# dcjones/polee

Hardware: AMD Instinct MI355X
Metric: approx-lik VI iters/sec (higher is better)
Workload: dtype f32

## Files before the change

### include/polee_hip_debug.h

```cpp
#ifndef POLEE_HIP_DEBUG_H
#define POLEE_HIP_DEBUG_H

#include "polee_hip.h"

#ifdef __cplusplus
extern "C" {
#endif

polee_status polee_debug_ptt_plan(const int32_t *node_parent_idxs, const int32_t *node_js, int32_t N,
                                  uint32_t *tour_code, int32_t *tour_tgt, int32_t *leaf_tid,
                                  int32_t *lo, int32_t *mid, int32_t *hi1, int32_t *max_depth);

typedef struct polee_psell_debug polee_psell_debug;
typedef struct {
    int64_t m, n, nnz, num_slices, num_tiles, padded_nnz, num_empty_rows;
    int64_t data_bytes, dict_len;
    int32_t max_row_nnz, max_tile_cols;
    const uint8_t *data;
    const uint32_t *slice_off;
    const uint32_t *tile_slice;
    const uint32_t *tile_dict;
    const uint32_t *dict;
    const uint32_t *row_order;
    const float *slice_ks;
    const uint8_t *slice_flags;
    int64_t num_tiles_a;
    int64_t num_tiles_a1;
    int64_t num_tiles_a1m;
    int64_t num_tiles_a2;
    const uint8_t *slice_w;
    int64_t num_tiles_s;
    int64_t stream_rows[8], stream_nnz[8], stream_bytes[8];
    int64_t csr_num_rows;
    const uint32_t *csr_rowptr;
    const uint32_t *csr_col;
    const float *csr_val;
    const uint32_t *csr_rows;
    int64_t single_num_rows;
    const uint32_t *single_rows;
    const float *single_cnt;
    double single_logsum;
} polee_psell_view;
polee_status polee_debug_psell_build(int64_t m, int64_t n, const void *colptr, int colptr_bytes,
                                     const uint32_t *rowval, const float *nzval,
                                     const int64_t *ks_or_null, polee_psell_debug **out);
polee_status polee_debug_psell_build_device(polee_ctx *ctx, int64_t m, int64_t n, const void *colptr, int colptr_bytes,
                                            const uint32_t *rowval, const float *nzval, const int64_t *ks_or_null,
                                            int device_stages, polee_psell_debug **out);
polee_status polee_debug_psell_view(const polee_psell_debug *p, polee_psell_view *view);
void polee_debug_psell_free(polee_psell_debug *p);

void polee_debug_device_cache_poison(int64_t *checked_blocks, int64_t *bad_blocks, int64_t *bad_words);

polee_status polee_debug_loglik_force_mixed(polee_loglik *ll, int on);

int64_t polee_debug_regression_num_stats(const polee_regression *reg);
polee_status polee_debug_regression_data_pass(polee_regression *reg, const float *noise, float *stats);
polee_status polee_debug_regression_prior_pass(polee_regression *reg, const float *stats, float *loss,
                                               float *grad_or_null);

polee_status polee_debug_comm_allreduce_ms(polee_comm *comm, int64_t count, int32_t reps, double *ms_avg);

polee_status polee_debug_fast_log(polee_ctx *ctx, const double *x, int64_t count, double *out);
polee_status polee_debug_fast_exp(polee_ctx *ctx, const double *x, int64_t count, double *out);

polee_status polee_debug_gibbs_assignments(polee_gibbs *g, int32_t chain, int32_t *z);

#ifdef __cplusplus
}
#endif
#endif
```

### polee_amd/csrc/loglik.hip

```cpp
#include "loglik_internal.hpp"
#include "psell_device.hpp"
#include "wave.hpp"

#include <algorithm>
#include <chrono>
#include <cmath>
#include <queue>
#include <type_traits>

namespace polee {

template <int CTRL, int ROW_MASK>
__device__ inline float dpp_mov0(float v)
{
    return __int_as_float(__builtin_amdgcn_update_dpp(0, __float_as_int(v), CTRL, ROW_MASK, 0xf, true));
}

template <int K>
__device__ inline void scatter_runs(int c, float (&q)[K], float *gw, int lane)
{
    const int c0 = __builtin_amdgcn_readfirstlane(c);
    if (__all(c == c0)) {
        float *gr = gw + c0 * K;
        wave_sum_to_lane63_n<K>(q);
// ... 66 lines not shown
    }
    __device__ inline void mul(float s, bool valid)
    {
        const float sv = valid ? s : 1.0f;
        const float p = m * __builtin_amdgcn_frexp_mantf(sv);
        m = __builtin_amdgcn_frexp_mantf(p);
        e += __builtin_amdgcn_frexp_expf(sv) + __builtin_amdgcn_frexp_expf(p);
    }
    __device__ inline double log_value() const { return ((double)e + (double)__builtin_amdgcn_logf(m)) * 0.693147180559945309417; }
};
__device__ inline double ks_log2(float ksv, float s) { return (double)(ksv * __builtin_amdgcn_logf(s)); }

struct PsellArgs {
    const uint8_t *data;
    const uint32_t *slice_off, *tile_slice, *tile_dict, *dict;
    const float *slice_ks;
    const float *x;
    float *g;
    double *lp;
    int lcap;
    int tiles_a;
    int tiles_a1;
    int tiles_a1m, tiles_a2;
    int tiles_s;
    const float *xwin;
    const PosDesc *sched;
    const PosDesc *sched_dyn;
    unsigned int *dyn_ctr;
    unsigned int dyn_base;
    unsigned int dyn_last;
    float *gwin;
    double *lpwin;
    int lp_slot0;
};

template <int K, bool WANT_LP, bool HAS_KS>
__device__ inline void psell_tile_body(const PsellArgs &A, int tile, float *xw, float *gw, double *lp_red)
{
    const uint8_t *__restrict__ data = A.data;
    const uint32_t *__restrict__ slice_off = A.slice_off;
    const uint32_t *__restrict__ tile_slice = A.tile_slice;
    const uint32_t *__restrict__ tile_dict = A.tile_dict;
    const uint32_t *__restrict__ dict = A.dict;
    const float *__restrict__ slice_ks = A.slice_ks;
    const float *__restrict__ x = A.x;
    float *__restrict__ g = A.g;
    double *__restrict__ lp = A.lp;

    const uint32_t d0 = tile_dict[tile];
    const int L = (int)(tile_dict[tile + 1] - d0);
    for (int i = threadIdx.x; i < L * K; i += 256) {
        const int l = i / K, k = i - l * K;
        xw[i] = x[(size_t)dict[d0 + l] * K + k];
        gw[i] = 0.0f;
    }
    __syncthreads();

    const int lane = threadIdx.x & 63, wave = threadIdx.x >> 6;
    const uint32_t s0 = tile_slice[tile], s1 = tile_slice[tile + 1];
    const bool compact = tile < A.tiles_a;
    double lpacc[K];
#pragma unroll
    for (int k = 0; k < K; ++k) lpacc[k] = 0.0;

    const int stream = tile < A.tiles_a1 ? PSELL_A1 : (tile < A.tiles_a1m ? PSELL_A1M : (tile < A.tiles_a2 ? PSELL_A2 : (tile < A.tiles_a ? PSELL_A2M : (tile < A.tiles_s ? PSELL_BN : PSELL_B))));
    const bool det = A.gwin != nullptr && tile >= A.tiles_s;
// ... 222 lines not shown
    return l;
}

__device__ inline void lds_barrier()
{
    asm volatile("s_waitcnt lgkmcnt(0)\n\ts_barrier" ::: "memory");
}

#ifdef POLEE_STAMPS
__device__ unsigned long long g_stamps[24];

#define STAMP(i)                                                          \
    do {                                                                  \
        const unsigned long long now__ = __builtin_amdgcn_s_memtime();    \
        st_acc[i] += now__ - st_last;                                     \
        st_last = now__;                                                  \
    } while (0)
#else
#define STAMP(i) do { } while (0)
#endif
#ifdef POLEE_TILE_CYCLES
__device__ unsigned long long g_tile_cycles[1 << 17];
__device__ unsigned long long g_wg_cycles[4096];
#endif
constexpr int NSTAMP = 16;

struct WaveStream {
    uint32_t ent;
    int nsl;
    int npieces;
    int issued, islot;
    int primed;
    const uint8_t *gsrc;
};

template <uint32_t RB>
__device__ inline void ring_refill(WaveStream &ws, uint32_t ring_lds, int target)
{
    constexpr int RP = (int)(RB / 1024u);
    int issued = __builtin_amdgcn_readfirstlane(ws.issued), islot = __builtin_amdgcn_readfirstlane(ws.islot);
    target = __builtin_amdgcn_readfirstlane(target);
    const uint32_t voff = (uint32_t)wave_lane() * 16u;
    const uint8_t *src = reinterpret_cast<const uint8_t *>(uniform_ptr(ws.gsrc + (size_t)issued * 1024));
    for (; issued < target; ++issued) {
        dma_1k(src, voff, ring_lds + (uint32_t)islot * 1024u);
        src += 1024;
        islot = islot + 1 == RP ? 0 : islot + 1;
    }
    ws.issued = issued;
    ws.islot = islot;
}

template <int K, uint32_t RB, bool WANT_LP, bool HAS_KS>
__device__ inline void wide_stream(WaveStream &ws, const char *ring, int extras, const float *xw, float *gw, double &lpacc, int dbg
#ifdef POLEE_STAMPS
                                   , unsigned long long (&st_acc)[NSTAMP], unsigned long long &st_last
#endif
                                   )
{
    constexpr int RP = (int)(RB / 1024u);
    constexpr uint32_t STAGE_A = 256u + 16u * 256u;
    static_assert(STAGE_A + 2046u <= RB && (PSELL_WIDE_MAX - 16 + 1) * 256u + 2046u <= RB, "a stage of a wide slice (+ ks row) must fit the ring");
    const int lane = wave_lane();
    const uint32_t ring_lds = lds_addr(ring);

    typedef float f32x4 __attribute__((ext_vector_type(4)));
    constexpr int NT = 2;
    constexpr int NS = 8;
    const int tt = lane & 15, q = lane >> 4;
    f32x4 acc0[NT], acc1[NT];
    uint2 colq[NT];
    float xq[NS];
#pragma unroll
    for (int mt = 0; mt < NT; ++mt) {
        acc0[mt] = f32x4{0.f, 0.f, 0.f, 0.f};
        acc1[mt] = f32x4{0.f, 0.f, 0.f, 0.f};
        colq[mt] = make_uint2(0u, 0u);
    }
#pragma unroll
    for (int st = 0; st < NS; ++st) xq[st] = 0.0f;
    int pend_w = 0;
    LogAcc lpl;
    lpl.init();
// ... 179 lines not shown
    const uint64_t E = 0x5555555555555555ull, L = 0x3333333333333333ull;
    asm volatile("s_nop 1\n\t"
                 "s_mov_b64 vcc, %8\n\t"
                 "v_cndmask_b32_dpp %4, %1, %0, vcc quad_perm:[1,0,3,2] row_mask:0xf bank_mask:0xf\n\t"
                 "v_cndmask_b32_dpp %6, %3, %2, vcc quad_perm:[1,0,3,2] row_mask:0xf bank_mask:0xf\n\t"
                 "s_not_b64 vcc, vcc\n\t"
                 "v_cndmask_b32_dpp %5, %0, %1, vcc quad_perm:[1,0,3,2] row_mask:0xf bank_mask:0xf\n\t"
                 "v_cndmask_b32_dpp %7, %2, %3, vcc quad_perm:[1,0,3,2] row_mask:0xf bank_mask:0xf\n\t"
                 "s_mov_b64 vcc, %9\n\t"
                 "v_cndmask_b32_dpp %0, %6, %4, vcc quad_perm:[2,3,0,1] row_mask:0xf bank_mask:0xf\n\t"
                 "v_cndmask_b32_dpp %1, %7, %5, vcc quad_perm:[2,3,0,1] row_mask:0xf bank_mask:0xf\n\t"
                 "s_not_b64 vcc, vcc\n\t"
                 "v_cndmask_b32_dpp %2, %4, %6, vcc quad_perm:[2,3,0,1] row_mask:0xf bank_mask:0xf\n\t"
                 "v_cndmask_b32_dpp %3, %5, %7, vcc quad_perm:[2,3,0,1] row_mask:0xf bank_mask:0xf"
                 : "+v"(a0), "+v"(a1), "+v"(a2), "+v"(a3), "=&v"(y0), "=&v"(y1), "=&v"(y2), "=&v"(y3)
                 : "s"(E), "s"(L)
                 : "vcc", "scc");
}

template <int K, uint32_t RB, bool WANT_LP, bool HAS_KS, bool MASKED>
__device__ inline void narrow_stream(WaveStream &ws, const char *ring, int extras, const float *xw, float *gw,
                                     uint32_t aux_lds, double &lpacc, int dbg
#ifdef POLEE_STAMPS
                                     , unsigned long long (&st_acc)[NSTAMP], unsigned long long &st_last
#endif
                                     )
{
    typedef float f32x4 __attribute__((ext_vector_type(4)));
    typedef const __attribute__((address_space(3))) float *lds_cfp;
    typedef __attribute__((address_space(3))) float *lds_fp;
    constexpr int WMAX = PSELL_NARROW_MAX;
    static_assert(WMAX == 16, "four groups of four transcripts");
    constexpr int KG = (K + 3) / 4;
    constexpr int RP = (int)(RB / 1024u);
    const int lane = wave_lane();
    const uint32_t ring_lds = lds_addr(ring);
    const uint32_t xw_lds = lds_addr(xw), gw_lds = lds_addr(gw);
    const int j = lane & 3, b = lane >> 2;
    const uint32_t j4 = 4u * (uint32_t)j;
    uint32_t lc1[4];
#pragma unroll
    for (int u = 0; u < 4; ++u) lc1[u] = ring_lds + ((uint32_t)(lane ^ u) << 2);
    const uint32_t j256 = 256u * (uint32_t)j;
    auto lds_f = [](uint32_t a) -> float { return *reinterpret_cast<lds_cfp>((uintptr_t)a); };
    auto wrap_u = [&](uint32_t a) -> uint32_t {
        a = (uint32_t)__builtin_amdgcn_readfirstlane((int)a);
        return a >= RB ? a - RB : a;
    };

    f32x4 acc[4][KG];
    float xq[8][KG];
#pragma unroll
    for (int g = 0; g < 4; ++g)
#pragma unroll
        for (int kg = 0; kg < KG; ++kg) acc[g][kg] = f32x4{0.f, 0.f, 0.f, 0.f};
#pragma unroll
    for (int t = 0; t < 8; ++t)
#pragma unroll
        for (int kg = 0; kg < KG; ++kg) xq[t][kg] = 0.0f;
    uint32_t xav = aux_lds, gav = aux_lds + 32u;
    int pend_w = 0;
    int run_w = 0;
    LogAcc lpl[KG];
    double lp2[KG];
#pragma unroll
    for (int kg = 0; kg < KG; ++kg) {
        lpl[kg].init();
// ... 6 lines not shown
        const uint32_t ga = ((lane & 32) ? ((lane & 16) ? ga3 : ga1) : ((lane & 16) ? ga2 : ga0)) + j4;
#pragma unroll
        for (int kg = 0; kg < KG; ++kg) {
            auto r1 = __builtin_amdgcn_permlane32_swap(__float_as_uint(acc[g][kg][0]), __float_as_uint(acc[g][kg][1]), false, false);
            const float ab = __uint_as_float(r1[0]) + __uint_as_float(r1[1]);
            auto r2 = __builtin_amdgcn_permlane32_swap(__float_as_uint(acc[g][kg][2]), __float_as_uint(acc[g][kg][3]), false, false);
            const float cd = __uint_as_float(r2[0]) + __uint_as_float(r2[1]);
            auto r3 = __builtin_amdgcn_permlane16_swap(__float_as_uint(ab), __float_as_uint(cd), false, false);
            float q = __uint_as_float(r3[0]) + __uint_as_float(r3[1]);
            q += __int_as_float(__builtin_amdgcn_update_dpp(0, __float_as_int(q), 0x114, 0xf, 0xf, true));
            q += __int_as_float(__builtin_amdgcn_update_dpp(0, __float_as_int(q), 0x118, 0xf, 0xf, true));
            if ((lane & 12) == 12 && 4 * kg + j < K && !(dbg & 2))
                __hip_atomic_fetch_add(reinterpret_cast<lds_fp>((uintptr_t)(ga + 16u * (uint32_t)kg)), q, __ATOMIC_RELAXED,
                                       __HIP_MEMORY_SCOPE_WORKGROUP);
            acc[g][kg] = f32x4{0.f, 0.f, 0.f, 0.f};
        }
    };
    auto flush = [&]() {
        flush_group(0);
        if (pend_w > 4) flush_group(1);
        if (pend_w > 8) flush_group(2);
        if (pend_w > 12) flush_group(3);
        pend_w = 0;
    };
    auto load_x_group = [&](int g, float (*dst)[KG]) {
#pragma unroll
        for (int u = 0; u < 4; ++u) {
            const uint32_t a = (uint32_t)__builtin_amdgcn_readlane((int)xav, 4 * g + u) + j4;
            dst[u][0] = lds_f(a);
            if (KG > 1) dst[u][KG > 1 ? 1 : 0] = lds_f(a + 16u);
        }
    };

    uint32_t pos = 0;
    uint32_t pos_r = 0;
    for (int si = 0; si < ws.nsl; ++si) {
        const uint32_t e0 = (uint32_t)__builtin_amdgcn_readlane((int)ws.ent, si);
        const uint32_t e1 = (uint32_t)__builtin_amdgcn_readlane((int)ws.ent, si + 1);
        const uint32_t off = e0 & PSELL_OFF_MASK, off_next = e1 & PSELL_OFF_MASK;
        const int flags = (int)(e0 >> 30);
        const uint32_t units = off_next - off;
        const int nrows = (int)(units / 2u) - 1 - (HAS_KS ? 1 : 0);
        int w = MASKED ? run_w : nrows;
        const uint32_t bytes = units * 128u;
        if (!(dbg & 16)) __builtin_amdgcn_s_setprio(3);
        STAMP(1);
        {
            const int need = (int)((pos + bytes + 1023u) >> 10);
            int allowed = ws.issued - need + (need <= ws.primed ? extras : 0);
            wait_vm_outstanding(__builtin_amdgcn_readfirstlane(allowed));
        }
        STAMP(2);
        if (pend_w != 0 && !(flags & 2)) flush();
        if (pend_w == 0 && !((dbg & 64) && si > 0)) {
            const uint32_t cid = *reinterpret_cast<const __attribute__((address_space(3))) uint16_t *>(
                (uintptr_t)(ring_lds + pos_r + (MASKED ? 4u * (uint32_t)(lane & 15) + 2u : 2u * (uint32_t)(lane & 15))));
            const bool live = MASKED ? cid != (uint32_t)PSELL_NO_COL : (lane & 15) < w;
            if (MASKED) {
                run_w = __builtin_popcount((uint32_t)__ballot(live) & 0xffffu);
                w = run_w;
            }
            xav = live ? xw_lds + cid * (uint32_t)(K * 4) : aux_lds;
            gav = live ? gw_lds + cid * (uint32_t)(K * 4) : aux_lds + 32u;
            load_x_group(0, xq);
            if (w > 4) load_x_group(1, xq + 4);
        }
        STAMP(3);

        const uint32_t row0 = wrap_u(pos_r + 256u);
        f32x4 d1[KG];
#pragma unroll
        for (int kg = 0; kg < KG; ++kg) d1[kg] = f32x4{ROWSUM_FLOOR, ROWSUM_FLOOR, ROWSUM_FLOOR, ROWSUM_FLOOR};
        f32x4 kv = f32x4{1.f, 1.f, 1.f, 1.f};
        auto consumed = [&]() {
            asm volatile("s_waitcnt lgkmcnt(0)" ::: "memory");
            STAMP(11);
            pos += bytes;
            pos_r += bytes;
            pos_r = pos_r >= RB ? pos_r - RB : pos_r;
            ring_refill<RB>(ws, ring_lds, min(ws.npieces, (int)(pos >> 10) + RP));
            STAMP(6);
            if (!(dbg & 16)) __builtin_amdgcn_s_setprio(0);
        };
        auto body = [&](auto NGc, auto FASTc) {
            constexpr int NG = decltype(NGc)::value;
            constexpr bool FAST = decltype(FASTc)::value;
            float pv[8], qv[2][4];
            uint32_t bp[4];
            if (FAST) {
#pragma unroll
                for (int u = 0; u < 4; ++u) bp[u] = lc1[u] + pos_r;
            }
            auto read_p = [&](int g0, int g1) {
#pragma unroll
                for (int g = g0; g < g1; ++g) {
                    if (FAST) {
#pragma unroll
                        for (int u = 0; u < 4; ++u) pv[4 * (g - g0) + u] = lds_f(bp[u] + 256u + 1024u * (uint32_t)g + 256u * (uint32_t)u);
                    } else {
                        const uint32_t rg = wrap_u(row0 + 1024u * (uint32_t)g);
#pragma unroll
                        for (int u = 0; u < 4; ++u) pv[4 * (g - g0) + u] = lds_f(lc1[u] + wrap_u(rg + 256u * (uint32_t)u));
                    }
                }
            };
            auto read_q = [&](int g0, int g1) {
#pragma unroll
                for (int g = g0; g < g1; ++g) {
                    if (FAST) {
#pragma unroll
                        for (int u = 0; u < 4; ++u) qv[g - g0][u] = lds_f(bp[u] + j256 + 256u + 1024u * (uint32_t)g);
                    } else {
                        const uint32_t rg = wrap_u(row0 + 1024u * (uint32_t)g);
// ... 81 lines not shown
                for (int u = 0; u < 8; ++u) pw[u] = pv[u];
                read_p(2, NG);
                if (!(dbg & 4)) {
                    load_x_group(2, xr);
                    if (NG > 3) load_x_group(3, xr + 4);
                } else {
#pragma unroll
                    for (int u = 0; u < 8; ++u)
#pragma unroll
                        for (int kg = 0; kg < KG; ++kg) xr[u][kg] = xq[u][kg];
                }
                asm volatile("s_waitcnt lgkmcnt(0)" ::: "memory");
                if (!(dbg & 16)) __builtin_amdgcn_s_setprio(0);
                phase1(pw, xq);
                phase1(pw + 4, xq + 4);
                phase1(pv, xr);
                if (NG > 3) phase1(pv + 4, xr + 4);
                read_q(0, 2);
#pragma unroll
                for (int u = 0; u < 4; ++u) {
                    qw[0][u] = qv[0][u];
                    qw[1][u] = qv[1][u];
                }
                read_q(2, NG);
                weights();
                consumed();
                phase2(0, qw[0]);
                phase2(1, qw[1]);
                phase2(2, qv[0]);
                if (NG > 3) phase2(3, qv[1]);
            }
        };
        using std::integral_constant;
        const bool fast = pos_r + bytes <= RB;
        if (fast) {
            if (w <= 4) body(integral_constant<int, 1>(), integral_constant<bool, true>());
            else if (w <= 8) body(integral_constant<int, 2>(), integral_constant<bool, true>());
            else if (w <= 12) body(integral_constant<int, 3>(), integral_constant<bool, true>());
            else body(integral_constant<int, 4>(), integral_constant<bool, true>());
        } else {
            if (w <= 4) body(integral_constant<int, 1>(), integral_constant<bool, false>());
            else if (w <= 8) body(integral_constant<int, 2>(), integral_constant<bool, false>());
            else if (w <= 12) body(integral_constant<int, 3>(), integral_constant<bool, false>());
            else body(integral_constant<int, 4>(), integral_constant<bool, false>());
        }
        pend_w = w;
        STAMP(5);
    }
    if (pend_w != 0) flush();
    if (WANT_LP) {
#pragma unroll
        for (int kg = 0; kg < KG; ++kg) {
            double v = HAS_KS ? lp2[kg] * 0.693147180559945309417 : lpl[kg].log_value();
            v += __shfl_xor(v, 4, 64);
            v += __shfl_xor(v, 8, 64);
            v += __shfl_xor(v, 16, 64);
            v += __shfl_xor(v, 32, 64);
            if (lane < 16 && (lane >> 2) == kg && lane < K) lpacc += v;
        }
    }
}

template <int K>
__device__ inline void scatter_runs_lds(int c, float (&q)[K], uint32_t gw_lds, int lane)
{
    typedef __attribute__((address_space(3))) float *lds_fp;
    auto add = [](uint32_t a, float v) {
        __hip_atomic_fetch_add(reinterpret_cast<lds_fp>((uintptr_t)a), v, __ATOMIC_RELAXED, __HIP_MEMORY_SCOPE_WORKGROUP);
// ... 496 lines not shown
    for (int k = 0; k < PSELL_MAX_K; ++k) ls[k] = 0.0;
    if (c != 0.0f) {
        const float *xr = x + (size_t)j * K;
        float *gr = g + (size_t)j * K;
#pragma unroll
        for (int k = 0; k < PSELL_MAX_K; ++k)
            if (k < K) {
                const float xv = xr[k];
                if (g) gr[k] += c / xv;
                if (part) ls[k] = (double)c * log((double)xv);
            }
    }
    if (!part) return;
#pragma unroll
    for (int k = 0; k < PSELL_MAX_K; ++k) {
        double v = ls[k];
#pragma unroll
        for (int d = 32; d >= 1; d >>= 1) v += __shfl_down(v, d, 64);
        if ((threadIdx.x & 63) == 0) sm[threadIdx.x >> 6][k] = v;
    }
    __syncthreads();
    if (threadIdx.x < K) part[(size_t)blockIdx.x * K + threadIdx.x] = ((sm[0][threadIdx.x] + sm[1][threadIdx.x]) + sm[2][threadIdx.x]) + sm[3][threadIdx.x];
}
__global__ void single_lp_finish_kernel(const double *__restrict__ part, int nblocks, int K, double logsum, double *__restrict__ lp)
{
    const int k = threadIdx.x;
    if (k >= K) return;
    double s = logsum;
    for (int b = 0; b < nblocks; ++b) s += part[(size_t)b * K + k];
    lp[k] += s;
}

constexpr uint32_t STREAM_RB1 = 7168u, STREAM_RB2 = 14336u, STREAM_RINGS = 28672u;
template <int K>
constexpr uint32_t stream_ring_total()
{
    return STREAM_RINGS;
}
template <int K>
constexpr uint32_t stream_xw_bytes()
{
    return ((uint32_t)PSELL_TILE_COLS_TARGET * K * 4u + 1023u) & ~1023u;
}
template <int K, bool DET>
constexpr uint32_t stream_lds_bytes()
{
    return stream_ring_total<K>() + (DET ? 6u : 3u) * stream_xw_bytes<K>() + 2u * PSELL_TILE_COLS_TARGET * 4u + 4u * 256u + 2u * 256u + 64u;
}

template <int K, bool WANT_LP, bool HAS_KS, bool DET>
__global__ __launch_bounds__(256) __attribute__((amdgpu_waves_per_eu((WANT_LP || HAS_KS) ? 3 : 4, (WANT_LP || HAS_KS) ? 3 : 4)))
void loglik_stream_kernel(PsellArgs A, int dbg)
{
    extern __shared__ float lds[];
    constexpr uint32_t XWB = stream_xw_bytes<K>();
    constexpr uint32_t GWN = DET ? 4u : 1u;
    char *const base = reinterpret_cast<char *>(lds);
    char *const rings = base;
    auto xw_of = [&](int b) -> float * { return reinterpret_cast<float *>(base + stream_ring_total<K>() + (uint32_t)b * XWB); };
    float *const gw = reinterpret_cast<float *>(base + stream_ring_total<K>() + 2 * XWB);
    auto ids_of = [&](int b) -> uint32_t * {
        return reinterpret_cast<uint32_t *>(base + stream_ring_total<K>() + (2 + GWN) * XWB + (uint32_t)b * (PSELL_TILE_COLS_TARGET * 4));
    };
    uint32_t *const entb = reinterpret_cast<uint32_t *>(base + stream_ring_total<K>() + (2 + GWN) * XWB + 2 * PSELL_TILE_COLS_TARGET * 4);
    uint32_t *const descb = entb + 4 * 64;
    float *const auxz = reinterpret_cast<float *>(descb + 2 * 64);
// ... 12 lines not shown
#ifdef POLEE_TILE_CYCLES
    const unsigned long long t_wg0 = __builtin_amdgcn_s_memtime();
    unsigned long long t_tile0 = t_wg0;
#endif

    auto kind_of = [&](uint32_t tile) -> int { return (int)tile < A.tiles_a1 ? 0 : ((int)tile < A.tiles_a1m ? 2 : ((int)tile < A.tiles_a2 ? 1 : ((int)tile < A.tiles_a ? 3 : 4))); };
    auto share = [&](int kind, const PosDesc &t, uint32_t &sb, uint32_t &se) {
        const int nw = kind == 3 ? 2 : 4;
        uint32_t a1 = t.c1, a2 = t.c2, a3 = t.c3;
        asm volatile("" : "+s"(a1), "+s"(a2), "+s"(a3));
        const uint32_t lo = wave == 0 ? t.s0 : (wave == 1 ? a1 : (wave == 2 ? a2 : a3));
        const uint32_t hi = wave + 1 >= nw ? t.s1 : (wave == 0 ? a1 : (wave == 1 ? a2 : a3));
        sb = wave < nw ? lo : t.s1;
        se = wave < nw ? hi : t.s1;
    };
    auto prefetch = [&](const PosDesc &t, int buf) -> int {
        int cnt = 0;
        const int npx = (int)((t.L * (uint32_t)K * 4u + 1023u) >> 10);
        const uint8_t *src = xwin_b + (size_t)t.d0 * K * 4;
        const uint32_t dst = lds_addr(xw_of(buf));
        for (int p = wave; p < npx; p += 4) {
            dma_1k_keep(uniform_ptr(src + (size_t)p * 1024), (uint32_t)wave_lane() * 16u, dst + (uint32_t)p * 1024u);
            ++cnt;
        }
        if ((uint32_t)wave * 64u < t.L) {
            dma_256(uniform_ptr(A.dict + t.d0 + (uint32_t)wave * 64u), min((uint32_t)wave_lane(), t.L - 1u - (uint32_t)wave * 64u) * 4u,
                    lds_addr(ids_of(buf)) + (uint32_t)wave * 256u);
            ++cnt;
        }
        const int kind = kind_of(t.tile);
        {
            uint32_t sb, se;
            share(kind, t, sb, se);
            dma_256(uniform_ptr(A.slice_off + sb), min((uint32_t)wave_lane(), se - sb) * 4u, lds_addr(entb) + (uint32_t)wave * 256u);
            ++cnt;
        }
        return cnt;
    };
    WaveStream ws;
    const int ahead = (dbg >> 8) & 15;
    auto start_ring = [&](const PosDesc &t) {
        const int kind = kind_of(t.tile);
        ws.nsl = 0; ws.npieces = 0; ws.issued = 0; ws.islot = 0; ws.primed = 0; ws.ent = 0u; ws.gsrc = A.data;
        uint32_t sb, se;
        share(kind, t, sb, se);
        ws.ent = entb[wave * 64 + wave_lane()];
        ws.nsl = (int)(se - sb);
        const uint32_t cb = (uint32_t)__builtin_amdgcn_readlane((int)ws.ent, 0) & PSELL_OFF_MASK;
        const uint32_t ce = (uint32_t)__builtin_amdgcn_readlane((int)ws.ent, ws.nsl) & PSELL_OFF_MASK;
        ws.npieces = (int)(((ce - cb) * 128u + 1023u) >> 10);
        ws.gsrc = reinterpret_cast<const uint8_t *>(uniform_ptr(A.data + (size_t)cb * 128));
        if (kind != 3) {
            ring_refill<STREAM_RB1>(ws, lds_addr(rings + wave * STREAM_RB1), min(ws.npieces, ahead ? min(ahead, (int)(STREAM_RB1 / 1024u)) : (int)(STREAM_RB1 / 1024u)));
        } else {
            ring_refill<STREAM_RB2>(ws, lds_addr(rings + (wave < 2 ? wave : 0) * STREAM_RB2), min(ws.npieces, ahead ? min(2 * ahead, (int)(STREAM_RB2 / 1024u)) : (int)(STREAM_RB2 / 1024u)));
        }
        ws.primed = ws.issued;
    };

    double lp_a = 0.0;

    PosDesc cur = sched[blockIdx.x];
    if (cur.tile == POS_NONE) return;
    PosDesc nxt = sched[blockIdx.x + G];
    for (int i = threadIdx.x; i < (int)(GWN * XWB / 4u); i += 256) gw[i] = 0.0f;
    for (int i = threadIdx.x; i < (int)(stream_ring_total<K>() / 16u); i += 256)
        reinterpret_cast<float4 *>(rings)[i] = make_float4(0.f, 0.f, 0.f, 0.f);
    if (threadIdx.x < 16) auxz[threadIdx.x] = 0.0f;
    lds_barrier();
    (void)prefetch(cur, 0);
    asm volatile("s_waitcnt vmcnt(0)" ::: "memory");
    start_ring(cur);
    int young = 0;
    lds_barrier();
    int buf = 0;
    for (uint32_t round = 0;; ++round) {
        const bool more = nxt.tile != POS_NONE;
        const int kind = kind_of(cur.tile);
        if (more) young += prefetch(nxt, buf ^ 1);
        if (wave == 0) {
// ... 162 lines not shown
{
    cut[0] = cut[1] = cut[2] = s1;
    if (t >= h.num_tiles_s) return;
    static const bool bytes_cut = getenv("POLEE_BYTES_CUT") != nullptr;
    const int nw = h.stream_of_tile(t) != PSELL_A2M ? 4 : 2;
    static const char *cut_env = getenv("POLEE_CUT_MODEL");
    static double cm[3] = {0, 0, 0};
    static const bool cut_custom = cut_env && sscanf(cut_env, "%lf,%lf,%lf", &cm[0], &cm[1], &cm[2]) == 3;
    auto cost = [&](uint32_t sl) {
        const int w = h.slice_w[sl];
        if (bytes_cut) return 512.0 + 128.0 * (double)((h.slice_off[sl + 1] & PSELL_OFF_MASK) - (h.slice_off[sl] & PSELL_OFF_MASK));
        if (h.stream_of_tile(t) == PSELL_BN) return 6.0 * w + 4.0;
        if (cut_custom) {
            const double ng = (double)((w + 3) / 4);
            const bool cont = (h.slice_flags[sl] & 2) != 0 && sl > s0;
            return cm[0] + cm[1] * ng + (cont ? 0.0 : cm[2] * (1.0 + ng));
        }
        return 4.0 * ((w + 3) / 4) + (w <= 8 ? 8.0 : 16.0 * ((w + 15) / 16)) + 10.0;
    };
    double total = 0.0;
    for (uint32_t sl = s0; sl < s1; ++sl) total += cost(sl);
    double acc = 0.0;
    int wv = 1;
    for (uint32_t sl = s0; sl < s1 && wv < nw; ++sl) {
        acc += cost(sl);
        while (wv < nw && (acc >= total * wv / nw || sl + 1 - (wv == 1 ? s0 : cut[wv - 2]) >= 63u)) cut[wv++ - 1] = sl + 1;
    }
    if (s1 - (nw > 1 ? cut[nw - 2] : s0) > 63u) {
        const uint32_t per = (s1 - s0 + (uint32_t)nw - 1) / (uint32_t)nw;
        for (int q = 1; q < nw; ++q) cut[q - 1] = std::min(s1, s0 + per * (uint32_t)q);
    }
}

static polee_status ensure_schedule(polee_loglik *ll, int G)
{
    if (ll->sched_grid == G && ll->d_sched.p) return POLEE_OK;
    const PsellHost &h = ll->host;
    std::vector<uint32_t> order;
    order.reserve((size_t)h.num_tiles_s);
    for (int64_t t = 0; t < h.num_tiles_s; ++t) order.push_back((uint32_t)t);
    std::stable_sort(order.begin(), order.end(), [&](uint32_t a, uint32_t b) { return ll->tile_cost[a] > ll->tile_cost[b]; });
    std::vector<std::vector<uint32_t>> lists((size_t)G);
    {
        typedef std::pair<double, int> Load;
        std::priority_queue<Load, std::vector<Load>, std::greater<Load>> heap;
        for (int b = 0; b < G; ++b) heap.push(Load(0.0, b));
        for (uint32_t t : order) {
            Load l = heap.top();
            heap.pop();
            lists[(size_t)l.second].push_back(t);
            l.first += (double)ll->tile_cost[t];
            heap.push(l);
        }
    }
    size_t rounds = 0;
    for (auto &l : lists) rounds = std::max(rounds, l.size());
    std::vector<PosDesc> sched((rounds + 3) * (size_t)G);
    for (auto &d : sched) {
        d = PosDesc();
        d.tile = POS_NONE;
    }
    for (int b = 0; b < G; ++b) {
        std::vector<uint32_t> big, small;
        for (uint32_t t : lists[b]) (h.stream_of_tile(t) != PSELL_A2 && h.stream_of_tile(t) != PSELL_A2M ? big : small).push_back(t);
        const size_t n = big.size() + small.size();
        size_t ib = 0, is = 0;
        for (size_t j = 0; j < n; ++j) {
            const size_t want = ((j + 1 + (size_t)(b % 3)) * small.size()) / (n + 2);
            const bool take_small = (is < small.size()) && (ib >= big.size() || is < want);
            const uint32_t t = take_small ? small[is++] : big[ib++];
// ... 48 lines not shown
        std::copy(plist.begin(), plist.end(), dynl.begin());
        ll->dyn_pad = dynl.size() - plist.size();
        POLEE_TRY(ll->d_sched_dyn.upload(ll->ctx, dynl));
        std::vector<unsigned int> zero(2, 0u);
        POLEE_TRY(ll->d_dyn_ctr.upload(ll->ctx, zero));
    }
    return POLEE_OK;
}

template <int K, bool LP, bool KS, bool DET>
static polee_status launch_stream(polee_loglik *ll, PsellArgs &A, int dbg)
{
    polee_ctx *ctx = ll->ctx;
    const PsellHost &h = ll->host;
    hipStream_t st = ctx->stream;
    static_assert((PSELL_NARROW_MAX + 2) * 256 + 1024 <= STREAM_RB1, "A1 slices (+ ks row) must fit their ring");
    static_assert(((PSELL_MIXED_NARROW_MAX * 384 + 255) & ~255) + 256 + 1024 <= STREAM_RB1, "BN slices (+ ks row) must fit their ring");
    static_assert((PSELL_WIDE_MAX + 3) * 256 + 1024 <= STREAM_RB2, "A2M slices (+ ks row) must fit their ring");
    const size_t lds = stream_lds_bytes<K, DET>();
    int &occ = ll->occ_cache[K][LP ? 1 : 0][KS ? 1 : 0][DET ? 1 : 0];
    if (occ == 0) {
        int nb = 0;
        POLEE_HIP_TRY(ctx, hipOccupancyMaxActiveBlocksPerMultiprocessor(&nb, loglik_stream_kernel<K, LP, KS, DET>, 256, lds));
        occ = std::max(1, std::min(nb, 4));
        if (getenv("POLEE_DEBUG_PRINT"))
            fprintf(stderr, "[loglik] stream kernel K=%d%s: %d workgroups per CU by the occupancy query, LDS %zu B, grid %d x %d\n",
                    K, DET ? " (deterministic)" : "", nb, lds, occ, ctx->num_cus);
    }
    static const int wg_env = getenv("POLEE_STREAM_WGS_PER_CU") ? atoi(getenv("POLEE_STREAM_WGS_PER_CU")) : 0;
    const int per_cu = wg_env > 0 ? std::min(wg_env, occ) : occ;
    const int G = (int)std::min<int64_t>((int64_t)per_cu * ctx->num_cus, std::max<int64_t>(h.num_tiles_s, 1));
    POLEE_TRY(ensure_schedule(ll, G));
    A.sched = ll->d_sched.p;
    static const bool static_sched = getenv("POLEE_STATIC_SCHED") != nullptr;
    static const bool det_static = getenv("POLEE_DET_STATIC") != nullptr;
    if (!(DET && (LP || det_static)) && !static_sched && (size_t)3 * (size_t)G + 8 <= ll->dyn_pad) {
        A.sched_dyn = ll->d_sched_dyn.p;
        A.dyn_ctr = ll->d_dyn_ctr.p;
        A.dyn_base = ll->dyn_base;
        A.dyn_last = (unsigned int)(ll->dyn_positions + ll->dyn_pad - 1);
        ll->dyn_base += (uint32_t)ll->dyn_positions;
    }
    if (!ll->xwin_ready) {
        const bool side = ll->side_part != nullptr && !ll->side_done;
        hipLaunchKernelGGL((xwin_gather_kernel<K>), dim3((unsigned)ceil_div(ll->dict_len, 256) + (side ? 1u : 0u)), dim3(256), 0, st, A.dict,
                           A.x, ll->dict_len, ll->d_xwin.p, side ? ll->side_part : nullptr, ll->side_nparts, ll->side_out);
        if (side) ll->side_done = true;
    }
    if (ll->cur_e0) (void)hipEventRecord(ll->cur_e0, st);
    hipLaunchKernelGGL((loglik_stream_kernel<K, LP, KS, DET>), dim3((unsigned)G), dim3(256), lds, st, A, dbg);
    if (ll->cur_e1) (void)hipEventRecord(ll->cur_e1, st);
    A.lp_slot0 = G;
    return POLEE_OK;
}

template <int K, bool LP, bool KS>
static polee_status launch_variant(polee_loglik *ll, const float *d_x, float *d_g, double *d_lp)
{
    polee_ctx *ctx = ll->ctx;
    const PsellHost &h = ll->host;
    const int lcap_all = std::max(h.max_tile_cols, 1);
    hipStream_t st = ctx->stream;
    static const bool no_ring_env = getenv("POLEE_NO_RING") != nullptr;
    const bool no_ring = no_ring_env || ll->force_mixed;
    static const int dbg = getenv("POLEE_DBG_ABLATE") ? atoi(getenv("POLEE_DBG_ABLATE")) : 0;
    const LoglikRemap *rm = ll->cur_remap;
// ... 367 lines not shown
    val.resize(nnz);
    lap("allocate rows");
    parallel_chunks(B, 1, [&](size_t blo, size_t bhi, unsigned) {
        std::vector<uint32_t> local;
        for (size_t b = blo; b < bhi; ++b) {
            const uint64_t r0 = (uint64_t)b << sh, r1 = std::min<uint64_t>((uint64_t)m, r0 + ((uint64_t)1 << sh));
            local.assign((size_t)(r1 - r0) + 1, 0);
            for (uint64_t p = bstart[b]; p < bstart[b + 1]; ++p) ++local[stage[p].row - r0 + 1];
            for (size_t i = 1; i < local.size(); ++i) local[i] += local[i - 1];
            for (uint64_t i = 0; i < r1 - r0; ++i) rowptr[r0 + i + 1] = bstart[b] + local[i + 1];
            for (uint64_t p = bstart[b]; p < bstart[b + 1]; ++p) {
                const Rec &e = stage[p];
                const uint64_t q = bstart[b] + local[e.row - r0]++;
                col[q] = e.col;
                val[q] = e.val;
            }
        }
    });
    rowptr[0] = 0;
    lap("place within buckets");
    return "";
}
}

extern "C" {

polee_status polee_loglik_set_deterministic(polee_loglik *ll, int on)
{
    if (!ll) return fail(nullptr, POLEE_ERR_BAD_ARG, "null handle");
    ll->deterministic = on != 0;
    return POLEE_OK;
}

polee_status polee_debug_loglik_force_mixed(polee_loglik *ll, int on)
{
    if (!ll) return fail(nullptr, POLEE_ERR_BAD_ARG, "null handle");
    ll->force_mixed = on != 0;
    return POLEE_OK;
}

static polee_status loglik_create_on_device(polee_ctx *ctx, const PsellDevIn &X, bool has_ks, polee_loglik **out, bool &done)
{
    done = false;
    polee_loglik *ll = new (std::nothrow) polee_loglik();
    if (!ll) return fail(ctx, POLEE_ERR_OOM, "out of host memory");
    ll->ctx = ctx;
    ctx_retain(ctx);
    ll->m = X.m;
    ll->n = X.n;
    ll->has_ks = has_ks;
    PsellDevOut D;
    bool needs_host = false;
    polee_status st = psell_device_build(ctx, X, ll->host, D, false, needs_host);
    if (st != POLEE_OK || needs_host) {
        loglik_release(ll);
        return st;
    }
    ll->nnz = ll->host.nnz;
    ll->device_built = true;
    ll->d_data.take(D.data);
    if (has_ks) ll->d_slice_ks.take(D.slice_ks);
    done = true;
    return loglik_finish_create(ctx, ll, out);
}

static polee_status polee_loglik_create_from_xt_impl(polee_ctx *ctx, int64_t m, int64_t n, const uint64_t *tcolptr,
// ... 339 lines not shown
```

### polee_amd/csrc/loglik_internal.hpp

```cpp
#pragma once
#include "common.hpp"

namespace polee {

constexpr int PSELL_LANES = 64;
constexpr int PSELL_MAX_TILE_COLS = 1024;
constexpr int PSELL_TILE_COLS_TARGET = 128;
constexpr int PSELL_DICT_ALIGN = 4;
constexpr int PSELL_TILE_SLICES_A1 = 64;
constexpr int PSELL_TILE_SLICES_A2 = 32;
constexpr int PSELL_TILE_SLICES_B = 16;
constexpr int PSELL_MAX_K = 8;
constexpr uint32_t PSELL_OFF_MASK = 0x1fffffffu;
constexpr uint32_t PSELL_FLAG_MASKED_BIT = 29;
constexpr int PSELL_NARROW_MAX = 16;
constexpr int PSELL_WIDE_MAX = 32;
enum : int { PSELL_A1 = 0, PSELL_A1M = 1, PSELL_A2 = 2, PSELL_A2M = 3, PSELL_BN = 4, PSELL_B = 5, PSELL_C = 6, PSELL_S = 7, PSELL_NSTREAMS = 8 };
constexpr int PSELL_MIXED_NARROW_MAX = 15;
constexpr int PSELL_TILE_SLICES_A2M = 16;
constexpr int PSELL_TILE_SLICES_BN = 64;
constexpr uint32_t psell_row_pos(int stream, uint32_t t, uint32_t r) { return stream == PSELL_A1 ? (r ^ (t & 3u)) : (stream == PSELL_A2 ? ((r + 4u * t) & 63u) : r); }
constexpr uint16_t PSELL_NO_COL = 0x8000u;
constexpr uint32_t PSELL_PACK_CHUNK = 1u << 11;
constexpr uint32_t PSELL_MIXED_SEG_ROWS = 1u << 12;
constexpr double PSELL_PACK_WIDE_RESERVE = 32768.0;
constexpr int PSELL_MIN_UNIFORM_ROWS = 32;
constexpr int PSELL_MIN_UNION_ROWS = 1;

struct PosDesc {
    uint32_t tile;
    uint32_t s0, s1;
    uint32_t d0, L;
    uint32_t c1, c2, c3;
};
constexpr uint32_t POS_NONE = 0xffffffffu;

struct PsellHost {
    int64_t m = 0, n = 0, nnz = 0;
    int64_t num_slices = 0, num_tiles = 0, padded_nnz = 0, empty_rows = 0;
    int64_t rows_a = 0, num_tiles_a = 0, num_slices_a = 0;
    int64_t rows_a1 = 0, num_tiles_a1 = 0;
    int64_t rows_a1m = 0, num_tiles_a1m = 0;
    int64_t rows_a2 = 0, num_tiles_a2 = 0;
    int64_t rows_s = 0, num_tiles_s = 0;
    int64_t stream_rows[PSELL_NSTREAMS] = {}, stream_nnz[PSELL_NSTREAMS] = {}, stream_bytes[PSELL_NSTREAMS] = {};
    int stream_of_tile(int64_t t) const
    {
        return t < num_tiles_a1 ? PSELL_A1 : (t < num_tiles_a1m ? PSELL_A1M : (t < num_tiles_a2 ? PSELL_A2 : (t < num_tiles_a ? PSELL_A2M : (t < num_tiles_s ? PSELL_BN : PSELL_B))));
    }
    int32_t max_row = 0, max_tile_cols = 0;
    std::vector<uint8_t, default_init_allocator<uint8_t>> data;
    std::vector<uint32_t> slice_off;
    std::vector<uint32_t> tile_slice;
    std::vector<uint32_t> tile_dict;
    std::vector<uint32_t> tile_cols;
    std::vector<uint32_t> dict;
    std::vector<uint32_t> big_tiles;
    std::vector<uint8_t> slice_flags;
    std::vector<uint8_t> slice_w;
    std::vector<float> slice_ks;
    std::vector<uint32_t> row_order;
    std::vector<uint32_t> csr_rowptr;
    std::vector<uint32_t> csr_col, csr_rows;
    std::vector<float> csr_val, csr_ks;
    std::vector<float> single_cnt;
    double single_logsum = 0.0;
    std::vector<uint32_t> single_rows;
};
// ... 47 lines not shown
    polee_ctx *ctx = nullptr;
    int refs = 1;
    int64_t m = 0, n = 0, nnz = 0;
    bool has_ks = false;
    bool device_built = false;
    bool force_mixed = false;
    bool xwin_ready = false;
    const double *side_part = nullptr;
    int side_nparts = 0;
    double *side_out = nullptr;
    bool side_done = false;
    polee::PsellHost host;
    polee::DevBuf<uint8_t> d_data;
    polee::DevBuf<uint32_t> d_slice_off, d_tile_slice, d_tile_dict, d_dict;
    polee::DevBuf<float> d_slice_ks;
    polee::DevBuf<uint32_t> d_csr_rowptr;
    polee::DevBuf<uint32_t> d_csr_col;
    polee::DevBuf<float> d_csr_val, d_csr_ks;
    int64_t csr_rows = 0, csr_nnz = 0;
    polee::DevBuf<float> d_single_cnt;
    polee::DevBuf<double> d_single_part;
    bool has_singles = false;
    const polee::LoglikRemap *cur_remap = nullptr;
    polee::DevBuf<float> d_xwin;
    polee::DevBuf<polee::PosDesc> d_sched;
    int sched_grid = 0;
    polee::DevBuf<polee::PosDesc> d_sched_dyn;
    polee::DevBuf<unsigned int> d_dyn_ctr;
    size_t dyn_pad = 0;
    size_t dyn_positions = 0;
    uint32_t dyn_base = 0;
    std::vector<float> tile_cost;
    std::vector<uint32_t> tile_cut;
    int64_t dict_len = 0;
    int occ_cache[polee::PSELL_MAX_K + 1][2][2][2] = {};
    bool deterministic = false;
    polee::DevBuf<float> d_gwin;
    polee::DevBuf<double> d_lpwin;
    polee::DevBuf<uint32_t> d_tslot_ptr, d_tslot, d_theavy;
    polee::DevBuf<float> d_x_rows, d_x_aos, d_g_aos;
    polee::DevBuf<double> d_g_rows, d_lp;
    bool profile = false;
    int prof_every = 1;
    uint64_t prof_tick = 0;
    hipEvent_t cur_e0 = nullptr, cur_e1 = nullptr;
    hipEvent_t cur_p0 = nullptr, cur_p1 = nullptr;
    std::vector<hipEvent_t> prof_events;
    size_t prof_used = 0;
    int64_t prof_launches = 0;
    double prof_ms_total = 0.0, prof_pass_ms_total = 0.0;
    polee_status profile_collect();
};

namespace polee {
void loglik_retain(polee_loglik *ll);
void loglik_release(polee_loglik *ll);
polee_status loglik_eval_device(polee_loglik *ll, const float *d_x, int K, float *d_g, double *d_lp, bool xwin_ready = false,
                                const LoglikRemap *remap = nullptr);
}
```

Baseline: 2587.

## Precompute per-slice ring descriptors on host for narrow stream DMA scheduling

Builds a per-slice descriptor array on the host that packs ring position, wrap flag, row count, continuation bit, vmcnt wait value and refill count for the narrow stream kernels. The kernels read these descriptors instead of computing offsets, wait thresholds and refill targets from slice offsets at run time, and issue ring DMA with a simpler incremental issue routine. This is meant to cut scalar work and dependency chains in the narrow slice loop. In exchange there is an extra device buffer and a host build step, and the code fails with an unsupported error for slices that do not fit the bit fields.

```diff
diff --git a/include/polee_hip_debug.h b/include/polee_hip_debug.h
--- a/include/polee_hip_debug.h
+++ b/include/polee_hip_debug.h
@@ -54,6 +54,9 @@
 
 polee_status polee_debug_loglik_force_mixed(polee_loglik *ll, int on);
 
+polee_status polee_debug_slice_desc(const uint32_t *slice_off, int64_t num_slices, const uint32_t *tile_slice,
+                                    int64_t num_tiles_narrow, const uint32_t *tile_cut, uint32_t *out);
+
 int64_t polee_debug_regression_num_stats(const polee_regression *reg);
 polee_status polee_debug_regression_data_pass(polee_regression *reg, const float *noise, float *stats);
 polee_status polee_debug_regression_prior_pass(polee_regression *reg, const float *stats, float *loss,
diff --git a/polee_amd/csrc/loglik.hip b/polee_amd/csrc/loglik.hip
--- a/polee_amd/csrc/loglik.hip
+++ b/polee_amd/csrc/loglik.hip
@@ -122,6 +122,8 @@
     float *gwin;
     double *lpwin;
     int lp_slot0;
+    const uint32_t *sdesc = nullptr;
+    uint32_t sdesc_head = 0;
 };
 
 template <int K, bool WANT_LP, bool HAS_KS>
@@ -410,6 +412,8 @@
     int issued, islot;
     int primed;
     const uint8_t *gsrc;
+    const uint8_t *src;
+    uint32_t dst;
 };
 
 template <uint32_t RB>
@@ -427,6 +431,37 @@
     }
     ws.issued = issued;
     ws.islot = islot;
+}
+
+__device__ inline void dma_1k_salu_base(const void *base_uniform, uint32_t voff, uint32_t lds_dst)
+{
+    asm volatile("s_mov_b32 m0, %2\n\ts_nop 0\n\tglobal_load_lds_dwordx4 %1, %0" POLEE_DMA_POLICY
+                 :
+                 : "s"(base_uniform), "v"(voff), "s"(lds_dst)
+                 : "memory");
+}
+template <uint32_t RB>
+__device__ inline void ring_issue(WaveStream &ws, uint32_t ring_lds, int n)
+{
+    if (n <= 0) return;
+    const uint32_t voff = (uint32_t)wave_lane() * 16u;
+    const uint8_t *src = reinterpret_cast<const uint8_t *>(uniform_ptr(ws.src));
+    uint32_t dst = (uint32_t)__builtin_amdgcn_readfirstlane((int)ws.dst);
+    const uint32_t end = ring_lds + RB;
+    dma_1k(src, voff, dst);
+    for (int j = 1; j < n; ++j) {
+        src += 1024;
+        dst += 1024u;
+        dst = dst == end ? ring_lds : dst;
+#ifdef POLEE_DMA_BUILTIN
+        dma_1k(src, voff, dst);
+#else
+        dma_1k_salu_base(src, voff, dst);
+#endif
+    }
+    dst += 1024u;
+    ws.src = src + 1024;
+    ws.dst = dst == end ? ring_lds : dst;
 }
 
 template <int K, uint32_t RB, bool WANT_LP, bool HAS_KS>
@@ -672,7 +707,6 @@
     constexpr int WMAX = PSELL_NARROW_MAX;
     static_assert(WMAX == 16, "four groups of four transcripts");
     constexpr int KG = (K + 3) / 4;
-    constexpr int RP = (int)(RB / 1024u);
     const int lane = wave_lane();
     const uint32_t ring_lds = lds_addr(ring);
     const uint32_t xw_lds = lds_addr(xw), gw_lds = lds_addr(gw);
@@ -745,26 +779,17 @@
         }
     };
 
-    uint32_t pos = 0;
-    uint32_t pos_r = 0;
+    static_assert(RB == SDESC_RING, "slice descriptors describe the 7 KiB ring");
     for (int si = 0; si < ws.nsl; ++si) {
-        const uint32_t e0 = (uint32_t)__builtin_amdgcn_readlane((int)ws.ent, si);
-        const uint32_t e1 = (uint32_t)__builtin_amdgcn_readlane((int)ws.ent, si + 1);
-        const uint32_t off = e0 & PSELL_OFF_MASK, off_next = e1 & PSELL_OFF_MASK;
-        const int flags = (int)(e0 >> 30);
-        const uint32_t units = off_next - off;
-        const int nrows = (int)(units / 2u) - 1 - (HAS_KS ? 1 : 0);
+        const uint32_t sd = (uint32_t)__builtin_amdgcn_readlane((int)ws.ent, si);
+        const uint32_t pos_r = sd & SDESC_POS_MASK;
+        const int nrows = (int)((sd >> SDESC_ROWS_SHIFT) & 31u) - 1 - (HAS_KS ? 1 : 0);
         int w = MASKED ? run_w : nrows;
-        const uint32_t bytes = units * 128u;
         if (!(dbg & 16)) __builtin_amdgcn_s_setprio(3);
         STAMP(1);
-        {
-            const int need = (int)((pos + bytes + 1023u) >> 10);
-            int allowed = ws.issued - need + (need <= ws.primed ? extras : 0);
-            wait_vm_outstanding(__builtin_amdgcn_readfirstlane(allowed));
-        }
+        wait_vm_outstanding(__builtin_amdgcn_readfirstlane((int)((sd >> SDESC_WAIT_SHIFT) & 15u) + ((sd & SDESC_PRIMED_BIT) ? extras : 0)));
         STAMP(2);
-        if (pend_w != 0 && !(flags & 2)) flush();
+        if (pend_w != 0 && !(sd & SDESC_CONT_BIT)) flush();
         if (pend_w == 0 && !((dbg & 64) && si > 0)) {
             const uint32_t cid = *reinterpret_cast<const __attribute__((address_space(3))) uint16_t *>(
                 (uintptr_t)(ring_lds + pos_r + (MASKED ? 4u * (uint32_t)(lane & 15) + 2u : 2u * (uint32_t)(lane & 15))));
@@ -788,10 +813,7 @@
         auto consumed = [&]() {
             asm volatile("s_waitcnt lgkmcnt(0)" ::: "memory");
             STAMP(11);
-            pos += bytes;
-            pos_r += bytes;
-            pos_r = pos_r >= RB ? pos_r - RB : pos_r;
-            ring_refill<RB>(ws, ring_lds, min(ws.npieces, (int)(pos >> 10) + RP));
+            ring_issue<RB>(ws, ring_lds, (int)((sd >> SDESC_REFILL_SHIFT) & 15u));
             STAMP(6);
             if (!(dbg & 16)) __builtin_amdgcn_s_setprio(0);
         };
@@ -939,8 +961,7 @@
             }
         };
         using std::integral_constant;
-        const bool fast = pos_r + bytes <= RB;
-        if (fast) {
+        if (!(sd & SDESC_WRAP_BIT)) {
             if (w <= 4) body(integral_constant<int, 1>(), integral_constant<bool, true>());
             else if (w <= 8) body(integral_constant<int, 2>(), integral_constant<bool, true>());
             else if (w <= 12) body(integral_constant<int, 3>(), integral_constant<bool, true>());
@@ -1503,6 +1524,7 @@
 }
 
 constexpr uint32_t STREAM_RB1 = 7168u, STREAM_RB2 = 14336u, STREAM_RINGS = 28672u;
+static_assert(STREAM_RB1 == SDESC_RING, "the slice descriptors describe the narrow streams' ring");
 template <int K>
 constexpr uint32_t stream_ring_total()
 {
@@ -1581,7 +1603,10 @@
         {
             uint32_t sb, se;
             share(kind, t, sb, se);
-            dma_256(uniform_ptr(A.slice_off + sb), min((uint32_t)wave_lane(), se - sb) * 4u, lds_addr(entb) + (uint32_t)wave * 256u);
+            const bool nar = kind == 0 || kind == 2;
+            const uint32_t l = (uint32_t)wave_lane();
+            dma_256(uniform_ptr((nar ? A.sdesc : A.slice_off) + sb), (nar && l == 63u ? A.sdesc_head : min(l, se - sb)) * 4u,
+                    lds_addr(entb) + (uint32_t)wave * 256u);
             ++cnt;
         }
         return cnt;
@@ -1590,11 +1615,19 @@
     const int ahead = (dbg >> 8) & 15;
     auto start_ring = [&](const PosDesc &t) {
         const int kind = kind_of(t.tile);
-        ws.nsl = 0; ws.npieces = 0; ws.issued = 0; ws.islot = 0; ws.primed = 0; ws.ent = 0u; ws.gsrc = A.data;
+        ws.nsl = 0; ws.npieces = 0; ws.issued = 0; ws.islot = 0; ws.primed = 0; ws.ent = 0u; ws.gsrc = A.data; ws.src = A.data; ws.dst = 0u;
         uint32_t sb, se;
         share(kind, t, sb, se);
         ws.ent = entb[wave * 64 + wave_lane()];
         ws.nsl = (int)(se - sb);
+        if (kind == 0 || kind == 2) {
+            const uint32_t hd = (uint32_t)__builtin_amdgcn_readlane((int)ws.ent, 63);
+            const uint32_t ring_lds = lds_addr(rings + wave * STREAM_RB1);
+            ws.src = reinterpret_cast<const uint8_t *>(uniform_ptr(A.data + (size_t)(hd & PSELL_OFF_MASK) * 128));
+            ws.dst = ring_lds;
+            ring_issue<STREAM_RB1>(ws, ring_lds, ws.nsl > 0 ? (int)(hd >> SDESC_HEAD_P_SHIFT) : 0);
+            return;
+        }
         const uint32_t cb = (uint32_t)__builtin_amdgcn_readlane((int)ws.ent, 0) & PSELL_OFF_MASK;
         const uint32_t ce = (uint32_t)__builtin_amdgcn_readlane((int)ws.ent, ws.nsl) & PSELL_OFF_MASK;
         ws.npieces = (int)(((ce - cb) * 128u + 1023u) >> 10);
@@ -1823,10 +1856,57 @@
     }
 }
 
+static bool build_slice_desc(const uint32_t *slice_off, int64_t num_slices, const uint32_t *tile_slice, int64_t num_tiles_narrow,
+                             const uint32_t *tile_cut, uint32_t *out)
+{
+    constexpr uint32_t RB = SDESC_RING;
+    constexpr int RP = (int)(RB / 1024u);
+    std::fill(out, out + 2 * num_slices + 1, 0u);
+    uint32_t *head = out + num_slices + 1;
+    for (int64_t t = 0; t < num_tiles_narrow; ++t) {
+        const uint32_t b[5] = {tile_slice[t], tile_cut[3 * t], tile_cut[3 * t + 1], tile_cut[3 * t + 2], tile_slice[t + 1]};
+        for (int wv = 0; wv < 4; ++wv) {
+            const uint32_t sb = b[wv], se = b[wv + 1];
+            if (se <= sb) continue;
+            if (se - sb > 63u) return false;
+            const uint32_t cb = slice_off[sb] & PSELL_OFF_MASK, ce = slice_off[se] & PSELL_OFF_MASK;
+            const int npieces = (int)(((uint64_t)(ce - cb) * 128u + 1023u) >> 10);
+            const int primed = std::min(npieces, RP);
+            head[sb] = cb | ((uint32_t)primed << SDESC_HEAD_P_SHIFT);
+            int issued = primed;
+            uint64_t pos = 0;
+            for (uint32_t s = sb; s < se; ++s) {
+                const uint32_t units = (slice_off[s + 1] & PSELL_OFF_MASK) - (slice_off[s] & PSELL_OFF_MASK);
+                const uint64_t bytes = (uint64_t)units * 128u;
+                const uint32_t pos_r = (uint32_t)(pos % RB);
+                const int need = (int)((pos + bytes + 1023u) >> 10);
+                pos += bytes;
+                const int target = std::min(npieces, (int)(pos >> 10) + RP);
+                const int refill = std::max(0, target - issued);
+                const int wait = issued - need;
+                if ((units & 1u) || units / 2u > 31u || wait < 0 || wait > 15 || refill > 15) return false;
+                out[s] = pos_r | (pos_r + bytes > RB ? SDESC_WRAP_BIT : 0u) | ((units / 2u) << SDESC_ROWS_SHIFT) |
+                         ((slice_off[s] >> 31) ? SDESC_CONT_BIT : 0u) | ((uint32_t)wait << SDESC_WAIT_SHIFT) |
+                         (need <= primed ? SDESC_PRIMED_BIT : 0u) | ((uint32_t)refill << SDESC_REFILL_SHIFT);
+                issued += refill;
+            }
+        }
+    }
+    return true;
+}
+
 static polee_status ensure_schedule(polee_loglik *ll, int G)
 {
     if (ll->sched_grid == G && ll->d_sched.p) return POLEE_OK;
     const PsellHost &h = ll->host;
+    if (!ll->d_sdesc.p) {
+        if (h.slice_off.size() != (size_t)h.num_slices + 1)
+            return fail(ll->ctx, POLEE_ERR_BAD_ARG, "slice descriptors: the slice offsets are no longer on the host");
+        std::vector<uint32_t> sd((size_t)(2 * h.num_slices + 1));
+        if (!build_slice_desc(h.slice_off.data(), h.num_slices, h.tile_slice.data(), h.num_tiles_a1m, ll->tile_cut.data(), sd.data()))
+            return fail(ll->ctx, POLEE_ERR_UNSUPPORTED, "slice descriptors: a narrow slice outside the descriptor format");
+        POLEE_TRY(ll->d_sdesc.upload(ll->ctx, sd));
+    }
     std::vector<uint32_t> order;
     order.reserve((size_t)h.num_tiles_s);
     for (int64_t t = 0; t < h.num_tiles_s; ++t) order.push_back((uint32_t)t);
@@ -1941,6 +2021,8 @@
     const int G = (int)std::min<int64_t>((int64_t)per_cu * ctx->num_cus, std::max<int64_t>(h.num_tiles_s, 1));
     POLEE_TRY(ensure_schedule(ll, G));
     A.sched = ll->d_sched.p;
+    A.sdesc = ll->d_sdesc.p;
+    A.sdesc_head = (uint32_t)h.num_slices + 1u;
     static const bool static_sched = getenv("POLEE_STATIC_SCHED") != nullptr;
     static const bool det_static = getenv("POLEE_DET_STATIC") != nullptr;
     if (!(DET && (LP || det_static)) && !static_sched && (size_t)3 * (size_t)G + 8 <= ll->dyn_pad) {
@@ -2374,6 +2456,14 @@
     return POLEE_OK;
 }
 
+polee_status polee_debug_slice_desc(const uint32_t *slice_off, int64_t num_slices, const uint32_t *tile_slice,
+                                    int64_t num_tiles_narrow, const uint32_t *tile_cut, uint32_t *out)
+{
+    if (!slice_off || !tile_slice || !out || num_slices < 0 || num_tiles_narrow < 0 || (num_tiles_narrow > 0 && !tile_cut))
+        return POLEE_ERR_BAD_ARG;
+    return polee::build_slice_desc(slice_off, num_slices, tile_slice, num_tiles_narrow, tile_cut, out) ? POLEE_OK : POLEE_ERR_UNSUPPORTED;
+}
+
 polee_status polee_debug_loglik_force_mixed(polee_loglik *ll, int on)
 {
     if (!ll) return fail(nullptr, POLEE_ERR_BAD_ARG, "null handle");
diff --git a/polee_amd/csrc/loglik_internal.hpp b/polee_amd/csrc/loglik_internal.hpp
--- a/polee_amd/csrc/loglik_internal.hpp
+++ b/polee_amd/csrc/loglik_internal.hpp
@@ -34,6 +34,10 @@
     uint32_t c1, c2, c3;
 };
 constexpr uint32_t POS_NONE = 0xffffffffu;
+
+constexpr uint32_t SDESC_RING = 7168u;
+constexpr uint32_t SDESC_POS_MASK = 0x1fffu, SDESC_WRAP_BIT = 1u << 13, SDESC_ROWS_SHIFT = 14, SDESC_CONT_BIT = 1u << 19;
+constexpr uint32_t SDESC_WAIT_SHIFT = 20, SDESC_PRIMED_BIT = 1u << 24, SDESC_REFILL_SHIFT = 25, SDESC_HEAD_P_SHIFT = 29;
 
 struct PsellHost {
     int64_t m = 0, n = 0, nnz = 0;
@@ -147,6 +151,7 @@
     uint32_t dyn_base = 0;
     std::vector<float> tile_cost;
     std::vector<uint32_t> tile_cut;
+    polee::DevBuf<uint32_t> d_sdesc;
     int64_t dict_len = 0;
     int occ_cache[polee::PSELL_MAX_K + 1][2][2][2] = {};
     bool deterministic = false;
```

After: 2618, median of 6. +1.2%, better.
